# tkortz/opencv

Hardware: AMD Instinct MI355X
Metric: tracked frames/sec, 1080p×128-object TBD loop @ 1/2/4/8 MI355X (higher is better)
Workload: dtype u8; 1 GPU; TBD loop 1920x1080 x 128 objects (BASELINE configs[2]), frames [5, 2577) of a 2577-frame sequence per GPU; levels=3, win=21, gftt=256/box, q 0.01, minDist 3, every 5, tracker_bounds=reference, parallelism=replicas x1 (one sequence per GPU), api=tbdk_tbd_run (native frame loop, look-ahead)

## Files before the change

opencv_amd/csrc/klt_gftt.hip:

```cpp
#include <atomic>
#include <cfloat>
#include <cmath>
#include <type_traits>

#include "klt_gftt_device.hpp"
#include "tbdk_internal.hpp"

namespace tbdk {

namespace {

__device__ __forceinline__ int refl(int p, int len)
{
    if ((unsigned)p < (unsigned)len) return p;
    if (len == 1) return 0;
    do {
        if (p < 0) p = -p;
        else p = 2 * len - 2 - p;
    } while ((unsigned)p >= (unsigned)len);
    return p;
}

}

__device__ __forceinline__ int roi_of_cblock(const GfttArgs& a, int b)
{
    int lo = 0, hi = a.nroi - 1;
    while (lo < hi) {
        const int mid = (lo + hi + 1) >> 1;
        if ((a.ninl > 0 ? a.inl[mid].cblk : a.rois[mid].cblk) <= b) lo = mid;
        else hi = mid - 1;
    }
    return lo;
}

__device__ __forceinline__ float from_left(float v)
{
    return __int_as_float(__builtin_amdgcn_mov_dpp(__float_as_int(v), 0x138, 0xF, 0xF, true));
}
__device__ __forceinline__ float from_right(float v)
{
    return __int_as_float(__builtin_amdgcn_mov_dpp(__float_as_int(v), 0x130, 0xF, 0xF, true));
}

struct SobelRow {
    float rx, ry;
};
__device__ __forceinline__ SobelRow sobel_row(float s0, float s1, float s2, float k, float k2)
{
    float t = -1.f * s0;
    t = t + 0.f * s1;
    t = t + 1.f * s2;
    float u = k * s0;
    u = u + k2 * s1;
    u = u + k * s2;
    return SobelRow{t, u};
}
__device__ __forceinline__ SobelRow sobel_row_f32(float s0, float s1, float s2, float k, float k2)
{
    return SobelRow{s2 - s0, s1 * k2 + (s0 + s2) * k};
}

#ifndef TBDK_GFTT_EIG_WAVES
#define TBDK_GFTT_EIG_WAVES 4
#endif
constexpr int kEigWaves = TBDK_GFTT_EIG_WAVES;
constexpr int kEigPref = 8;
#ifndef TBDK_GFTT_EIG_PREF_C
#define TBDK_GFTT_EIG_PREF_C 4
#endif
#ifndef TBDK_GFTT_WALK_PRIO
#define TBDK_GFTT_WALK_PRIO 3
#endif
#ifndef GFTT_ESTAMP
#define GFTT_ESTAMP(i)
#endif

struct EigLane {
    __amdgpu_buffer_rsrc_t rs;
    int x, H, hm2, pitch;
    bool mir, out_lane;
    float k, k2;
};

__device__ __forceinline__ uint32_t row_off(int row, int pitch) { return (uint32_t)row * (uint32_t)pitch; }

struct EigMask {
    __amdgpu_buffer_rsrc_t rs;
    uint32_t col;
    int pitch;
};
__device__ __forceinline__ bool eig_mask_ld(const EigMask& m, int row)
{
    return __builtin_amdgcn_raw_buffer_load_b8(m.rs, m.col, (int)row_off(row, m.pitch), 0) != 0;
}

template <int PX = TBDK_PIX_U8>
__device__ __forceinline__ float eig_ld(const EigLane& g, int row)
{
    if constexpr (PX == TBDK_PIX_F32)
        return __uint_as_float(__builtin_amdgcn_raw_buffer_load_b32(g.rs, g.x * 4, (int)row_off(row, g.pitch), 0));
    else if constexpr (PX == TBDK_PIX_U16)
        return (float)__builtin_amdgcn_raw_buffer_load_b16(g.rs, g.x * 2, (int)row_off(row, g.pitch), 0);
    else
        return (float)__builtin_amdgcn_raw_buffer_load_b8(g.rs, g.x, (int)row_off(row, g.pitch), 0);
}

template <int PX = TBDK_PIX_U8>
__device__ __forceinline__ SobelRow eig_srow(const EigLane& g, float v)
{
    const float l = from_left(v), rr = from_right(v);
    if constexpr (PX != TBDK_PIX_U8) return sobel_row_f32(g.mir ? rr : l, v, g.mir ? l : rr, g.k, g.k2);
    else return sobel_row(g.mir ? rr : l, v, g.mir ? l : rr, g.k, g.k2);
}

__device__ __forceinline__ void eig_rowsums(const EigLane& g, const SobelRow& p, const SobelRow& c,
                                            const SobelRow& n, double (&out)[3])
{
    const float dx = (p.rx + n.rx) * g.k + (c.rx * g.k2 + 0.f);
    const float dy = (n.ry - p.ry) + 0.f;
    const float cv[3] = {dx * dx, dx * dy, dy * dy};
#pragma unroll
    for (int ch = 0; ch < 3; ++ch) {
        const float l = from_left(cv[ch]), rr = from_right(cv[ch]);
        out[ch] = (double)l + (double)cv[ch] + (double)rr;
    }
}

template <bool compact, bool masked, int PREF = compact ? TBDK_GFTT_EIG_PREF_C : kEigPref, int PX = TBDK_PIX_U8>
__device__ __forceinline__ void eig_segment(const EigLane& g, const EigMask& gm, float* __restrict__ E,
                                            uint64_t* __restrict__ lm,
                                            int w, int ep, int y0, int y1, int ys, int ye, int ycap, bool fresh,
                                            double (&S)[3], double (&S0)[3], double (&Scap)[3], int& best, int ccol)
{
    const int H = g.H;
    auto pix = [&](int yy) { return eig_ld<PX>(g, refl(yy, H)); };
    auto pix_fwd = [&](int yy) { return eig_ld<PX>(g, yy < H ? yy : g.hm2); };
    const int lane = threadIdx.x & 63;
    const bool x_in = g.out_lane && g.x >= 1 && g.x <= w - 2;
    double qa[3], qb[3];
    {
        const int rm = refl(ys - 1, H);
        eig_rowsums(g, eig_srow<PX>(g, pix(rm - 1)), eig_srow<PX>(g, pix(rm)), eig_srow<PX>(g, pix(rm + 1)), qa);
    }
    SobelRow wa = eig_srow<PX>(g, pix(ys)), wb = eig_srow<PX>(g, pix(ys + 1));
    eig_rowsums(g, eig_srow<PX>(g, pix(ys - 1)), wa, wb, qb);
    if (fresh) {
#pragma unroll
        for (int ch = 0; ch < 3; ++ch) S[ch] = (0.0 + qa[ch]) + qb[ch];
    }
#pragma unroll
    for (int ch = 0; ch < 3; ++ch) S0[ch] = S[ch];
    float e1 = 0.f, e2 = 0.f;
    const __amdgpu_buffer_rsrc_t rE =
        __builtin_amdgcn_make_buffer_rsrc(E - g.x, (short)0, ep * H * 4, 0x00020000);
    const __amdgpu_buffer_rsrc_t rL = __builtin_amdgcn_make_buffer_rsrc(lm, (short)0, lm ? H * 8 : 0, 0x00020000);
    constexpr uint32_t kDrop = 0x80000000u;
    const uint32_t eoff = g.out_lane ? (uint32_t)g.x * 4u : kDrop;
    auto row = [&](auto steady, int y, float cur, bool has_next, bool store, bool lmx) {
        constexpr bool ST = decltype(steady)::value;
        bool m_in = true;
        if constexpr (masked) {
            if (ST || store) m_in = eig_mask_ld(gm, y);
        }
        double in[3];
        SobelRow wc = wb;
        if (ST || has_next) {
            wc = eig_srow<PX>(g, cur);
            eig_rowsums(g, wa, wb, wc, in);
        } else {
#pragma unroll
            for (int ch = 0; ch < 3; ++ch) in[ch] = qa[ch];
        }
        float box[3];
#pragma unroll
        for (int ch = 0; ch < 3; ++ch) {
            const double t = S[ch] + in[ch];
            box[ch] = (float)t;
            S[ch] = t - qa[ch];
            qa[ch] = qb[ch];
            qb[ch] = in[ch];
        }
        wa = wb;
        wb = wc;
        const float aa = box[0] * 0.5f, bb = box[1], cc = box[2] * 0.5f;
        const float t = aa - cc;
        const float e = (aa + cc) - sqrtf(bb * bb + t * t);
        if (ST || store) {
            if constexpr (!compact)
                __builtin_amdgcn_raw_buffer_store_b32(__float_as_uint(e), rE, eoff == kDrop ? kDrop : eoff + (uint32_t)(y * ep * 4), 0, 0);
            const int kk = fkey(e);
            if constexpr (masked) best = (g.out_lane && m_in && kk > best) ? kk : best;
            else best = (g.out_lane && kk > best) ? kk : best;
        }
        if (ST || lmx) {
            float m = fmaxf(e2, e);
            m = fmaxf(m, fmaxf(from_left(e2), from_right(e2)));
            m = fmaxf(m, fmaxf(from_left(e1), from_right(e1)));
            m = fmaxf(m, fmaxf(from_left(e), from_right(e)));
            const bool lmax = x_in && e1 >= m;
            const uint64_t bal = __ballot(lmax);
            typedef unsigned int u32x2 __attribute__((ext_vector_type(2)));
            const u32x2 bv = {(unsigned)bal, (unsigned)(bal >> 32)};
            __builtin_amdgcn_raw_buffer_store_b64(bv, rL, lane == 0 ? (uint32_t)((y - 1) * 8) : kDrop, 0, 0);
            if constexpr (compact) {
                const uint32_t rk =
                    __builtin_amdgcn_mbcnt_hi((unsigned)(bal >> 32), __builtin_amdgcn_mbcnt_lo((unsigned)bal, 0u));
                __builtin_amdgcn_raw_buffer_store_b32(__float_as_uint(e1), rE,
                                                      lmax ? (uint32_t)(((y - 1) * ep + ccol + (int)rk) * 4) : kDrop, 0, 0);
            }
        }
        e2 = e1;
        e1 = e;
    };
    auto generic = [&](int y) {
        if (y == ycap) {
#pragma unroll
            for (int ch = 0; ch < 3; ++ch) Scap[ch] = S[ch];
        }
        const int yc = y - 1;
        row(std::false_type{}, y, y + 1 < H ? pix_fwd(y + 2) : 0.f, y + 1 < H, y >= y0 && y < y1,
            yc >= y0 && yc < y1 && yc >= 1 && yc <= H - 2);
    };
    const int sa = max(max(y0 + 1, 2), ys);
    int sb = min(min(y1, H - 1), ye);
    if (ycap >= 0) sb = min(sb, ycap);
    int y = ys;
    if (sb - sa >= PREF) {
        for (; y < sa; ++y) generic(y);
        float nxt[PREF];
#pragma unroll
        for (int j = 0; j < PREF; ++j) nxt[j] = pix_fwd(y + 2 + j);
        for (; y + PREF <= sb; y += PREF) {
            float cur[PREF];
#pragma unroll
            for (int j = 0; j < PREF; ++j) cur[j] = nxt[j];
#pragma unroll
            for (int j = 0; j < PREF; ++j) nxt[j] = pix_fwd(min(y + PREF + 2 + j, H));
#pragma unroll
            for (int j = 0; j < PREF; ++j) row(std::true_type{}, y + j, cur[j], true, true, true);
        }
    }
    for (; y < ye; ++y) generic(y);
}

template <bool compact, bool masked, int PX = TBDK_PIX_U8>
__device__ __forceinline__ void gftt_eig_body(const GfttArgs& a)
{
    constexpr int kPref = compact ? TBDK_GFTT_EIG_PREF_C : kEigPref;
    constexpr int kBpp = PX == TBDK_PIX_F32 ? 4 : PX == TBDK_PIX_U16 ? 2 : 1;
    __shared__ double s_cap[kEigWaves][3][64];
    __shared__ double s_drift[3][64];
    __shared__ int s_best[kEigWaves];
    __shared__ int s_bad;
    const int r = roi_of_cblock(a, blockIdx.x);
    const GfttRoi R = roi_at(a, r);
    const int wv = __builtin_amdgcn_readfirstlane(threadIdx.x >> 6);
    const int lane = threadIdx.x & 63;
    const int H = R.h;

    EigLane g;
    const int strip = blockIdx.x - R.cblk;
    const int xc = strip * kGfttStrip - kGfttHalo + lane;
    g.out_lane = lane >= kGfttHalo && lane < kGfttHalo + kGfttStrip && xc < R.w;
    {
        const int w = R.w;
        int xm = xc < -2 || xc > w + 1 ? min(max(xc, 0), w - 1) : xc;
        if (w == 1) {
            xm = 0;
        } else {
#pragma unroll
            for (int it = 0; it < 2; ++it) {
                if (xm < 0) xm = -xm;
                if (xm >= w) xm = 2 * (w - 1) - xm;
            }
        }
        g.x = xm;
        g.mir = xc < 0 || xc >= w;
    }
    const double scale = PX == TBDK_PIX_U8 ? 1.0 / ((double)(1 << 2) * 3 * 255.0) : 1.0 / ((double)(1 << 2) * 3);
    g.k = (float)(1.0 * scale);
    g.k2 = (float)(2.0 * scale);
    g.H = H;
    g.hm2 = H >= 2 ? H - 2 : 0;
    g.pitch = a.pitch;
    g.rs = __builtin_amdgcn_make_buffer_rsrc(const_cast<uint8_t*>(a.img + (size_t)R.y * a.pitch + (size_t)R.x * kBpp),
                                             (short)0, (int)(row_off(H - 1, a.pitch) + (uint32_t)(R.w * kBpp)),
                                             0x00020000);
    EigMask gm{};
    if constexpr (masked) {
        gm.rs = __builtin_amdgcn_make_buffer_rsrc(const_cast<uint8_t*>(a.mask + (size_t)R.y * a.mask_pitch + R.x),
                                                  (short)0, (int)(row_off(H - 1, a.mask_pitch) + (uint32_t)R.w),
                                                  0x00020000);
        gm.col = g.out_lane ? (uint32_t)g.x : 0xFFFFFFFFu;
        gm.pitch = a.mask_pitch;
    }
    float* E = a.eig + R.off + g.x;
    uint64_t* lm = a.lmax + R.moff + (size_t)strip * H;
    const bool has_lm = R.w >= 3 && H >= 3;
    const int ccol = strip * kGfttStrip;

    const int L = (H + kEigWaves - 1) / kEigWaves;
    const int y0 = wv * L, y1 = min(H, y0 + L);
    const bool live = y0 < y1;
    const int ys = y0 > 0 ? y0 - 1 : 0, ye = min(H, y1 + 1);
    const int ycap = y1 < H ? y1 - 1 : -1;
    int best = INT_MIN;
    double S[3], S0[3], Scap[3];
    const bool need = lane >= kGfttHalo - 1 && lane <= kGfttHalo + kGfttStrip && xc >= 0 && xc < R.w;
    auto first_mismatch = [&](int from) {
        if (threadIdx.x == 0) s_bad = kEigWaves;
        __syncthreads();
        if (live && wv > from) {
            bool diff = a.eig_redo != 0 && wv == from + 1;
#pragma unroll
            for (int ch = 0; ch < 3; ++ch) diff |= need && S0[ch] != s_cap[wv - 1][ch][lane];
            if (__any(diff) && lane == 0) atomicMin(&s_bad, wv);
        }
        __syncthreads();
        return s_bad;
    };
    GFTT_ESTAMP(0);
    if (live) {
        eig_segment<compact, masked, kPref, PX>(g, gm, E, has_lm ? lm : nullptr, R.w, gftt_epitch(R.w), y0, y1, ys, ye,
                                                ycap, true, S, S0, Scap, best, ccol);
        if (ycap >= 0) {
#pragma unroll
            for (int ch = 0; ch < 3; ++ch) s_cap[wv][ch][lane] = Scap[ch];
        }
    }
    int bad = first_mismatch(0);
    GFTT_ESTAMP(1);
    while (bad < kEigWaves) {
        if (wv == bad && live) {
#pragma unroll
            for (int ch = 0; ch < 3; ++ch) s_drift[ch][lane] = s_cap[bad - 1][ch][lane] - S0[ch];
        }
        __syncthreads();
        if (wv >= bad && live) {
#pragma unroll
            for (int ch = 0; ch < 3; ++ch)
                S[ch] = wv == bad ? s_cap[bad - 1][ch][lane] : S0[ch] + s_drift[ch][lane];
        }
        __syncthreads();
        if (wv >= bad && live) {
            best = INT_MIN;
            eig_segment<compact, masked, kPref, PX>(g, gm, E, has_lm ? lm : nullptr, R.w, gftt_epitch(R.w), y0, y1, ys,
                                                    ye, ycap, false, S, S0, Scap, best, ccol);
            if (ycap >= 0) {
#pragma unroll
                for (int ch = 0; ch < 3; ++ch) s_cap[wv][ch][lane] = Scap[ch];
            }
        }
        bad = first_mismatch(bad);
    }
#pragma unroll
    for (int o = 32; o > 0; o >>= 1) {
        const int v = __shfl_xor(best, o);
        best = v > best ? v : best;
    }
    if (lane == 0) s_best[wv] = best;
    __syncthreads();
    GFTT_ESTAMP(2);
    if (threadIdx.x == 0) {
        int m = s_best[0];
#pragma unroll
        for (int k = 1; k < kEigWaves; ++k) m = s_best[k] > m ? s_best[k] : m;
        a.blk_max[blockIdx.x] = m;
    }
}

template <bool compact>
__global__ __launch_bounds__(64 * kEigWaves) void gftt_eig_kernel(GfttArgs a)
{
    gftt_eig_body<compact, false>(a);
}

template <bool compact>
__global__ __launch_bounds__(64 * kEigWaves) void gftt_eig_masked_kernel(GfttArgs a)
{
    gftt_eig_body<compact, true>(a);
}

template <bool compact, bool masked, int PX>
__global__ __launch_bounds__(64 * kEigWaves) void gftt_eigpx_kernel(GfttArgs a)
{
    static_assert(PX == TBDK_PIX_U16 || PX == TBDK_PIX_F32, "the 8-bit kernels are gftt_eig_kernel / gftt_eig_masked_kernel");
    gftt_eig_body<compact, masked, PX>(a);
}

#ifndef GFTT_STAMP
#define GFTT_STAMP(i)
#define GFTT_TDECL
#define GFTT_T(i)
#define GFTT_TDUMP
#endif

template <int J>
__device__ __forceinline__ int xor_lane(int v, int lane)
{
    if constexpr (J == 1) return __builtin_amdgcn_mov_dpp(v, 0xB1, 0xF, 0xF, true);
    else if constexpr (J == 2) return __builtin_amdgcn_mov_dpp(v, 0x4E, 0xF, 0xF, true);
    else if constexpr (J == 4 || J == 8) {
        const int up = __builtin_amdgcn_mov_dpp(v, 0x100 | J, 0xF, 0xF, true);
        const int dn = __builtin_amdgcn_mov_dpp(v, 0x110 | J, 0xF, 0xF, true);
        return (lane & J) ? dn : up;
    } else if constexpr (J == 16) return __builtin_amdgcn_ds_swizzle(v, 0x1F | (16 << 10));
    else return __shfl_xor(v, J);
}
template <int J>
__device__ __forceinline__ uint64_t xor_lane_u64(uint64_t v, int lane)
{
    const int lo = xor_lane<J>((int)(uint32_t)v, lane), hi = xor_lane<J>((int)(uint32_t)(v >> 32), lane);
    return ((uint64_t)(uint32_t)hi << 32) | (uint32_t)lo;
}

__device__ __forceinline__ void sort_keys_512(uint64_t* keys, int tid)
{
    static_assert(kSelThreads == 512, "eight runs of 64");
    const int lane = tid & 63, w = tid >> 6;
    uint64_t x = keys[tid];
    auto stage = [&](auto jc, int k) {
        constexpr int j = decltype(jc)::value;
        const uint64_t y = xor_lane_u64<j>(x, lane);
        const bool desc = (lane & k) == 0 || k == 64;
        const bool take_max = ((lane & j) == 0) == desc;
        x = take_max ? (x > y ? x : y) : (x < y ? x : y);
    };
    using I1 = std::integral_constant<int, 1>;
    using I2 = std::integral_constant<int, 2>;
    using I4 = std::integral_constant<int, 4>;
    using I8 = std::integral_constant<int, 8>;
    using I16 = std::integral_constant<int, 16>;
    using I32 = std::integral_constant<int, 32>;
    stage(I1{}, 2);
    stage(I2{}, 4), stage(I1{}, 4);
    stage(I4{}, 8), stage(I2{}, 8), stage(I1{}, 8);
    stage(I8{}, 16), stage(I4{}, 16), stage(I2{}, 16), stage(I1{}, 16);
    stage(I16{}, 32), stage(I8{}, 32), stage(I4{}, 32), stage(I2{}, 32), stage(I1{}, 32);
    stage(I32{}, 64), stage(I16{}, 64), stage(I8{}, 64), stage(I4{}, 64), stage(I2{}, 64), stage(I1{}, 64);
    keys[tid] = x;
    __syncthreads();
    int rank = lane;
    int pos[8];
    bool all[8];
#pragma unroll
    for (int r = 0; r < 8; ++r) {
        const uint64_t c = keys[r * 64 + 63];
        all[r] = r < w ? c >= x : c > x;
        pos[r] = 0;
    }
#pragma unroll
    for (int st = 32; st >= 1; st >>= 1) {
#pragma unroll
        for (int r = 0; r < 8; ++r) {
            const uint64_t c = keys[r * 64 + pos[r] + st - 1];
            const bool ahead = r < w ? c >= x : c > x;
            pos[r] += ahead ? st : 0;
        }
    }
#pragma unroll
    for (int r = 0; r < 8; ++r) rank += r != w ? (all[r] ? 64 : pos[r]) : 0;
    __syncthreads();
    keys[rank] = x;
    __syncthreads();
}

template <int RAD>
__device__ __forceinline__ void window_test(const uint8_t* img, int rw, int rh, int ix, int iy, float fx, float fy,
                                            int lane, double md2, bool& good, unsigned long long& inb)
{
    constexpr int NR = 2 * RAD + 1;
    constexpr bool THREE = NR + 7 > 16;
    constexpr uint64_t kHi = 0x8080808080808080ull, kLo7 = 0x7F7F7F7F7F7F7F7Full;
    const int x0 = ix - RAD;
    if constexpr (RAD <= 2) {
        uint64_t cv = 0;
#pragma unroll
        for (int t = 0; t < NR; ++t) {
            const int xx = x0 + t;
            cv |= ((xx >= 0 && xx < rw) ? 0xFFull : 0ull) << (8 * t);
        }
        uint64_t wv[NR];
        int sh[NR];
#pragma unroll
        for (int d = 0; d < NR; ++d) {
            const int yy = iy - RAD + d;
            const int yc = yy < 0 ? 0 : (yy >= rh ? rh - 1 : yy);
            const int base = yc * rw + x0;
            const int al = base > 0 ? (base & ~3) : 0;
            const uint32_t* wp = reinterpret_cast<const uint32_t*>(img + al);
            wv[d] = (uint64_t)wp[0] | ((uint64_t)wp[1] << 32);
            sh[d] = base - al;
        }
        uint64_t rej = 0;
#pragma unroll
        for (int d = 0; d < NR; ++d) {
            const int yy = iy - RAD + d;
            if (yy < 0 || yy >= rh) continue;
            uint64_t close = 0;
#pragma unroll
            for (int t = 0; t < NR; ++t) {
                const float ddx = (float)(t - RAD), ddy = (float)(d - RAD);
                close |= (((double)(ddx * ddx + ddy * ddy) < md2 && !(d == RAD && t == RAD)) ? 0xFFull : 0ull)
                         << (8 * t);
            }
            const uint64_t v = (sh[d] >= 0 ? wv[d] >> (8 * sh[d]) : wv[d] << (-8 * sh[d])) & cv & close;
            rej |= v & kHi;
            uint64_t nz = (((v & kLo7) + kLo7) | v) & ~v & kHi;
            while (nz) {
                const int t = __builtin_ctzll(nz) >> 3;
                nz &= nz - 1ull;
                const int c = (int)((v >> (8 * t)) & 0xFF);
                if (c - 1 < lane) inb |= 1ull << (c - 1);
            }
        }
        if (rej) good = false;
        (void)fx;
        (void)fy;
        return;
    }
    uint64_t cv_lo = 0, cv_hi = 0;
#pragma unroll
    for (int t = 0; t < NR; ++t) {
        const int xx = x0 + t;
        const uint64_t b = (xx >= 0 && xx < rw) ? 0xFFull : 0ull;
        if (t < 8) cv_lo |= b << (8 * t);
        else cv_hi |= b << (8 * (t - 8));
    }
    uint64_t w0[NR], w1[NR], w2[NR];
    int sh[NR];
#pragma unroll
    for (int d = 0; d < NR; ++d) {
        const int yy = iy - RAD + d;
        const int yc = yy < 0 ? 0 : (yy >= rh ? rh - 1 : yy);
        const int base = yc * rw + x0;
        const int al = base > 0 ? (base & ~7) : 0;
        const uint64_t* wp = reinterpret_cast<const uint64_t*>(img + al);
        w0[d] = wp[0];
        w1[d] = wp[1];
        w2[d] = THREE ? wp[2] : 0ull;
        sh[d] = base - al;
    }
    uint64_t rej = 0;
#pragma unroll
    for (int d = 0; d < NR; ++d) {
        const int yy = iy - RAD + d;
        if (yy < 0 || yy >= rh) continue;
        uint64_t close_lo = 0, close_hi = 0;
#pragma unroll
        for (int t = 0; t < NR; ++t) {
            const float ddx = (float)(t - RAD), ddy = (float)(d - RAD);
            const uint64_t b = ((double)(ddx * ddx + ddy * ddy) < md2 && !(d == RAD && t == RAD)) ? 0xFFull : 0ull;
            if (t < 8) close_lo |= b << (8 * t);
            else close_hi |= b << (8 * (t - 8));
        }
        uint64_t lo, hi;
        if (sh[d] >= 0) {
            const int b8 = 8 * sh[d];
            lo = sh[d] ? (w0[d] >> b8) | (w1[d] << (64 - b8)) : w0[d];
            hi = sh[d] ? (w1[d] >> b8) | (w2[d] << (64 - b8)) : w1[d];
        } else {
            const int b8 = -8 * sh[d];
            lo = w0[d] << b8;
            hi = (w1[d] << b8) | (w0[d] >> (64 - b8));
        }
        lo &= cv_lo & close_lo;
        hi &= cv_hi & close_hi;
        rej |= (lo | hi) & kHi;
        uint64_t nz_lo = (((lo & kLo7) + kLo7) | lo) & ~lo & kHi;
        uint64_t nz_hi = (((hi & kLo7) + kLo7) | hi) & ~hi & kHi;
        while (nz_lo | nz_hi) {
            int t;
            uint64_t src;
            if (nz_lo) {
                t = __builtin_ctzll(nz_lo) >> 3;
                nz_lo &= nz_lo - 1ull;
                src = lo;
            } else {
                t = __builtin_ctzll(nz_hi) >> 3;
                nz_hi &= nz_hi - 1ull;
                src = hi;
                t += 8;
            }
            const int v = (int)((src >> (8 * (t & 7))) & 0xFF);
            if (v - 1 < lane) inb |= 1ull << (v - 1);
        }
    }
    if (rej) good = false;
    (void)fx;
    (void)fy;
}

#ifndef TBDK_GFTT_PARTIAL
#define TBDK_GFTT_PARTIAL 1
#endif
constexpr int kSelTarget = 448;
constexpr int kSelRegs = 8;

__device__ uint64_t take_next64(uint64_t* rest, int nrest, int lane)
{
    uint64_t mine = 0ull;
    for (int c = 0; c < 64; ++c) {
        uint64_t best = 0ull;
        int bi = -1;
        for (int j = lane; j < nrest; j += 64) {
            const uint64_t v = rest[j];
            if (v > best) {
                best = v;
                bi = j;
            }
        }
        uint64_t m = best;
#pragma unroll
        for (int d = 32; d >= 1; d >>= 1) {
            const uint64_t o = shfl_xor_u64(m, d);
            m = o > m ? o : m;
        }
        if (m == 0ull) break;
        if (bi >= 0 && best == m) rest[bi] = 0ull;
        if (lane == c) mine = m;
        __builtin_amdgcn_s_waitcnt(0xC07F);
        __builtin_amdgcn_wave_barrier();
    }
    return mine;
}

template <int RMAX, bool masked = false>
__global__ __launch_bounds__(kSelThreads) void gftt_select_kernel(GfttArgs a)
{
    extern __shared__ __attribute__((aligned(16))) uint8_t smem[];
    uint64_t* keys = reinterpret_cast<uint64_t*>(smem);
    float2* acc = reinterpret_cast<float2*>(keys + a.cap);
    float2* bxy = acc + a.max_corners;
    uint8_t* img = reinterpret_cast<uint8_t*>(acc + ((a.max_corners + 65) & ~1));
    const int r = blockIdx.x;
    const GfttRoi R = roi_at(a, r);
    const int tid = threadIdx.x;
    __shared__ int s_total;
    GFTT_STAMP(0);
    const int area = R.w * R.h;
    const bool use_dist = a.min_distance >= 1.0;
    const double md2 = a.min_distance * a.min_distance;
    int rad = (int)ceil(a.min_distance) - 1;
    if ((double)(rad + 1) * (rad + 1) < md2) rad++;
    const bool img_mode = use_dist && area <= a.img_bytes && rad <= 6;
    if (img_mode)
        for (int i = tid * 16; i < area; i += kSelThreads * 16) *reinterpret_cast<uint4*>(img + i) = make_uint4(0, 0, 0, 0);

    const int nstrip = (R.w + kGfttStrip - 1) / kGfttStrip;
    const int nw = R.w >= 3 && R.h >= 3 ? nstrip * R.h : 0;
    const uint64_t word0 = tid < nw ? a.lmax[R.moff + tid] : 0ull;
    int mk = INT_MIN;
    {
        int b = R.cblk;
        const int e = R.cblk + nstrip;
        for (; b + 4 <= e; b += 4) {
            const int m0 = a.blk_max[b], m1 = a.blk_max[b + 1], m2 = a.blk_max[b + 2], m3 = a.blk_max[b + 3];
            mk = max(max(mk, max(m0, m1)), max(m2, m3));
        }
        for (; b < e; ++b) mk = a.blk_max[b] > mk ? a.blk_max[b] : mk;
    }
    const float roi_max = masked && mk == INT_MIN ? 0.f : fkey_inv(mk);
    const float thr = (float)((double)roi_max * a.quality);
    if (tid == 0) s_total = 0;
    __syncthreads();
    const float* Ep = a.eig + R.off;
    const uint8_t* Mp = masked ? a.mask + (size_t)R.y * a.mask_pitch + R.x : nullptr;
    if (R.w >= 3 && R.h >= 3) {
        if (thr > 0.f) {
            for (int wi = tid; wi < nw; wi += kSelThreads) {
                const int st = wi / R.h, y = wi - st * R.h;
                if (y < 1 || y > R.h - 2) continue;
                uint64_t word = wi == tid ? word0 : a.lmax[R.moff + wi];
                const float* Er = Ep + (size_t)y * gftt_epitch(R.w) + st * kGfttStrip - kGfttHalo;
                const float* Ec = Er + kGfttHalo;
                const uint8_t* Mr = masked ? Mp + (size_t)y * a.mask_pitch + st * kGfttStrip - kGfttHalo : nullptr;
                int rk = 0;
                while (word) {
                    int xs[8];
                    float vs[8];
                    [[maybe_unused]] uint8_t ms[8];
#pragma unroll
                    for (int u = 0; u < 8; ++u) {
                        xs[u] = -1;
                        if (word) {
                            xs[u] = __builtin_ctzll(word);
                            word &= word - 1ull;
                            vs[u] = a.compact ? Ec[rk++] : Er[xs[u]];
                            if constexpr (masked) ms[u] = Mr[xs[u]];
                        }
                    }
#pragma unroll
                    for (int u = 0; u < 8; ++u) {
                        bool in = xs[u] >= 0 && vs[u] > thr;
                        if constexpr (masked) in = in && ms[u] != 0;
                        if (in) {
                            const int q = atomicAdd(&s_total, 1);
                            if (q < a.cap) keys[q] = cand_key(vs[u], y, st * kGfttStrip + xs[u] - kGfttHalo);
                        }
                    }
                }
            }
        } else if (!a.compact) {
            const int iw = R.w - 2, n = iw * (R.h - 2), ep = gftt_epitch(R.w);
            for (int p = tid; p < n; p += kSelThreads) {
                const int y = p / iw + 1, x = p - (y - 1) * iw + 1;
                const float* Ec = Ep + (size_t)y * ep + x;
                const float v = Ec[0] > thr ? Ec[0] : 0.f;
                if (v == 0.f) continue;
                if constexpr (masked) {
                    if (Mp[(size_t)y * a.mask_pitch + x] == 0) continue;
                }
                float m = v;
#pragma unroll
                for (int dy = -1; dy <= 1; ++dy)
#pragma unroll
                    for (int dx = -1; dx <= 1; ++dx) {
                        const float q0 = Ec[dy * ep + dx];
                        const float q = q0 > thr ? q0 : 0.f;
                        m = q > m ? q : m;
                    }
                if (v == m) {
                    const int q = atomicAdd(&s_total, 1);
                    if (q < a.cap) keys[q] = cand_key(v, y, x);
                }
            }
        }
    }
    __syncthreads();
    GFTT_STAMP(4);
    const int total = s_total;
    if (total > a.cap) {
        if (tid == 0) a.counts[r] = -1;
        return;
    }
    int S = total, nrest = 0;
    if (TBDK_GFTT_PARTIAL && total > kSelThreads && total <= kSelRegs * kSelThreads && total + kSelThreads + 64 <= a.cap) {
        __shared__ int hist[256];
        __shared__ int s_pick[4];
        __shared__ int s_cnt[2];
        if (tid < 256) hist[tid] = 0;
        __syncthreads();
        for (int i = tid; i < total; i += kSelThreads) atomicAdd(&hist[(int)(keys[i] >> 56)], 1);
        __syncthreads();
        if (tid < 64) radix_pick(hist, kSelTarget, tid, &s_pick[0], &s_pick[1]);
        __syncthreads();
        const int b1 = s_pick[0], above1 = s_pick[1];
        if (tid < 256) hist[tid] = 0;
        __syncthreads();
        for (int i = tid; i < total; i += kSelThreads) {
            const uint64_t k = keys[i];
            if ((int)(k >> 56) == b1) atomicAdd(&hist[(int)(k >> 48) & 255], 1);
        }
        __syncthreads();
        if (tid < 64) {
            int b2 = -1, above2 = 0;
            radix_pick(hist, kSelTarget - above1, tid, &b2, &above2);
            if (b2 >= 0) {
                s_pick[2] = (b1 << 8) | b2;
                s_pick[3] = above1 + above2 + hist[b2];
            }
        }
        if (tid == 0) s_cnt[0] = s_cnt[1] = 0;
        __syncthreads();
        const int sel = s_pick[3];
        if (sel <= kSelThreads) {
            const uint32_t t16 = (uint32_t)s_pick[2];
            uint64_t kr[kSelRegs];
#pragma unroll
            for (int u = 0; u < kSelRegs; ++u) {
                const int i = tid + u * kSelThreads;
                kr[u] = i < total ? keys[i] : 0ull;
            }
            __syncthreads();
#pragma unroll
            for (int u = 0; u < kSelRegs; ++u) {
                if (tid + u * kSelThreads >= total) continue;
                if ((uint32_t)(kr[u] >> 48) >= t16) keys[atomicAdd(&s_cnt[0], 1)] = kr[u];
                else keys[kSelThreads + atomicAdd(&s_cnt[1], 1)] = kr[u];
            }
            __syncthreads();
            S = sel;
            nrest = total - sel;
        }
    }
    GFTT_STAMP(5);
    int np2 = kSelThreads;
    while (np2 < S) np2 <<= 1;
    for (int i = S + tid; i < np2; i += kSelThreads) keys[i] = 0ull;
    __syncthreads();
    GFTT_STAMP(1);
    switch (np2 / kSelThreads) {
    case 1: sort_keys_512(keys, tid); break;
    case 2: sort_keys<2>(keys, np2, tid); break;
    case 4: sort_keys<4>(keys, np2, tid); break;
    default: sort_keys_lds(keys, np2, tid); break;
    }
    GFTT_STAMP(2);
    if (tid >= 64) return;
    __builtin_amdgcn_s_setprio(TBDK_GFTT_WALK_PRIO);

    const int lane = tid;
    const int maxc = a.max_corners;
    float2* out = a.corners + (size_t)r * a.corner_stride;
    int n = 0;
    bool done = false;
    GFTT_TDECL;
    int i0 = 0, rem = nrest;
    while (!done) {
        GFTT_T(0);
        uint64_t key;
        bool valid;
        if (i0 < S) {
            const int i = i0 + lane;
            valid = i < S;
            key = valid ? keys[i] : 0ull;
            i0 += 64;
        } else {
            if (rem <= 0) break;
            key = take_next64(keys + kSelThreads, nrest, lane);
            valid = key != 0ull;
            rem -= 64;
        }
        const uint32_t kk = (uint32_t)key;
        const int ix = (int)(kk & 0xFFFF), iy = (int)(kk >> 16);
        const float fx = (float)ix, fy = (float)iy;
        bool good = valid;
        unsigned long long inb = 0ull;
        if (img_mode) {
            if (valid) img[iy * R.w + ix] = (uint8_t)(lane + 1);
            __builtin_amdgcn_s_waitcnt(0xC07F);
            __builtin_amdgcn_wave_barrier();
            GFTT_T(1);
            if (valid) {
                switch (rad) {
                case 0: window_test<0>(img, R.w, R.h, ix, iy, fx, fy, lane, md2, good, inb); break;
                case 1: window_test<1>(img, R.w, R.h, ix, iy, fx, fy, lane, md2, good, inb); break;
                case 2: window_test<2>(img, R.w, R.h, ix, iy, fx, fy, lane, md2, good, inb); break;
                default:
                    if constexpr (RMAX > 2) {
                        switch (rad) {
                        case 3: window_test<3>(img, R.w, R.h, ix, iy, fx, fy, lane, md2, good, inb); break;
                        case 4: window_test<4>(img, R.w, R.h, ix, iy, fx, fy, lane, md2, good, inb); break;
                        case 5: window_test<5>(img, R.w, R.h, ix, iy, fx, fy, lane, md2, good, inb); break;
                        default: window_test<6>(img, R.w, R.h, ix, iy, fx, fy, lane, md2, good, inb); break;
                        }
                    }
                    break;
                }
            }
        } else if (use_dist) {
            bxy[lane] = make_float2(fx, fy);
            for (int q = 0; q < n && good; ++q) {
                const float2 pq = acc[q];
                const float dx = fx - pq.x, dy = fy - pq.y;
                if ((double)(dx * dx + dy * dy) < md2) good = false;
            }
            __builtin_amdgcn_s_waitcnt(0xC07F);
            __builtin_amdgcn_wave_barrier();
            for (int j = 0; j < lane; ++j) {
                const float2 pj = bxy[j];
                const float dx = fx - pj.x, dy = fy - pj.y;
                if ((double)(dx * dx + dy * dy) < md2) inb |= 1ull << j;
            }
        }
        GFTT_T(2);
        const unsigned long long goodm = __ballot(good);
        const unsigned long long depm = __ballot(good && inb != 0ull);
        unsigned long long accm = goodm & ~depm;
        unsigned long long pend = depm;
        while (pend) {
            const int k = __builtin_ctzll(pend);
            pend &= pend - 1ull;
            const unsigned long long ik =
                ((unsigned long long)(uint32_t)__builtin_amdgcn_readlane((int)(inb >> 32), k) << 32) |
                (uint32_t)__builtin_amdgcn_readlane((int)(uint32_t)inb, k);
            if (!(ik & accm)) accm |= 1ull << k;
        }
        GFTT_T(3);
        const int got = __popcll(accm);
        if (n + got >= maxc) {
            int keepn = maxc - n;
            unsigned long long m = accm, t = 0ull;
            while (keepn-- > 0) {
                const unsigned long long low = m & (~m + 1ull);
                t |= low;
                m &= m - 1ull;
            }
            accm = t;
            done = true;
        }
        GFTT_T(4);
        const bool mine = (accm >> lane) & 1ull;
        if (mine) {
            const int pos = n + __popcll(accm & ((1ull << lane) - 1ull));
            if (!img_mode) acc[pos] = make_float2(fx, fy);
            out[pos] = make_float2(fx + (float)R.x, fy + (float)R.y);
        }
        if (img_mode && valid) img[iy * R.w + ix] = mine ? (uint8_t)255 : (uint8_t)0;
        n += __popcll(accm);
        __builtin_amdgcn_s_waitcnt(0xC07F);
        __builtin_amdgcn_wave_barrier();
        GFTT_T(5);
    }
    GFTT_TDUMP;
    GFTT_STAMP(3);
    if (lane == 0) a.counts[r] = n;
}

size_t gftt_select_smem(int cap, int max_corners, int img_bytes)
{
    return sizeof(uint64_t) * (size_t)cap +
           sizeof(float2) * (size_t)((max_corners + 65) & ~1) + (size_t)img_bytes + 32;
}

void gftt_plan(GfttArgs& a, int max_area)
{
    const long lds = 160L * 1024 - 2048;
    const long fixed = (long)gftt_select_smem(0, a.max_corners, 0);
    long img = ((long)max_area + 15) & ~15L;
    long room = lds - fixed - img;
    if (room < 8L * 4096) {
        img = 0;
        room = lds - fixed;
    }
    int cap = 512;
    while (cap < kGfttCap && 8L * cap * 2 <= room) cap <<= 1;
    a.cap = cap;
    a.img_bytes = (int)img;
}

template <int PX>
static void launch_gftt_eigpx(const GfttArgs& a, dim3 grid, dim3 block, hipStream_t s)
{
    if (a.mask) {
        if (a.compact) hipLaunchKernelGGL((gftt_eigpx_kernel<true, true, PX>), grid, block, 0, s, a);
        else hipLaunchKernelGGL((gftt_eigpx_kernel<false, true, PX>), grid, block, 0, s, a);
    } else {
        if (a.compact) hipLaunchKernelGGL((gftt_eigpx_kernel<true, false, PX>), grid, block, 0, s, a);
        else hipLaunchKernelGGL((gftt_eigpx_kernel<false, false, PX>), grid, block, 0, s, a);
    }
}

hipError_t launch_gftt_eig(const GfttArgs& a, hipStream_t s, int pix)
{
    const dim3 grid(a.ncblk), block(64 * kEigWaves);
    if (pix == TBDK_PIX_F32) {
        launch_gftt_eigpx<TBDK_PIX_F32>(a, grid, block, s);
    } else if (pix == TBDK_PIX_U16) {
        launch_gftt_eigpx<TBDK_PIX_U16>(a, grid, block, s);
    } else if (a.mask) {
        if (a.compact) hipLaunchKernelGGL(gftt_eig_masked_kernel<true>, grid, block, 0, s, a);
        else hipLaunchKernelGGL(gftt_eig_masked_kernel<false>, grid, block, 0, s, a);
    } else {
        if (a.compact) hipLaunchKernelGGL(gftt_eig_kernel<true>, grid, block, 0, s, a);
        else hipLaunchKernelGGL(gftt_eig_kernel<false>, grid, block, 0, s, a);
    }
    return hipGetLastError();
}

hipError_t launch_gftt(const GfttArgs& a, hipStream_t s, hipEvent_t after_eig, int pix, bool select)
{
    const hipError_t e0 = launch_gftt_eig(a, s, pix);
    if (e0 != hipSuccess) return e0;
    if (after_eig) {
        const hipError_t e = hipEventRecord(after_eig, s);
        if (e != hipSuccess) return e;
    }
    return select ? launch_gftt_select(a, s) : hipSuccess;
}

hipError_t launch_gftt_select(const GfttArgs& a, hipStream_t s)
{
    const size_t smem = gftt_select_smem(a.cap, a.max_corners, a.img_bytes);
    static std::atomic<unsigned long long> opted{0};
    int dev = 0;
    hipError_t e = hipGetDevice(&dev);
    if (e != hipSuccess) return e;
    const unsigned long long bit = 1ull << (dev & 63);
    if (!(opted.load(std::memory_order_acquire) & bit)) {
        for (const void* k : {reinterpret_cast<const void*>(&gftt_select_kernel<2>),
                              reinterpret_cast<const void*>(&gftt_select_kernel<6>),
                              reinterpret_cast<const void*>(&gftt_select_kernel<2, true>),
                              reinterpret_cast<const void*>(&gftt_select_kernel<6, true>)}) {
            hipFuncAttributes fa;
            e = hipFuncGetAttributes(&fa, k);
            if (e != hipSuccess) return e;
            e = hipFuncSetAttribute(k, hipFuncAttributeMaxDynamicSharedMemorySize,
                                    (int)(160L * 1024 - (long)fa.sharedSizeBytes));
            if (e != hipSuccess) return e;
        }
        opted.fetch_or(bit, std::memory_order_acq_rel);
    }
    const double md2 = a.min_distance * a.min_distance;
    int rad = (int)ceil(a.min_distance) - 1;
    if ((double)(rad + 1) * (rad + 1) < md2) rad++;
    const bool wide = a.min_distance >= 1.0 && rad > 2;
    if (a.mask) {
        if (wide) hipLaunchKernelGGL((gftt_select_kernel<6, true>), dim3(a.nroi), dim3(kSelThreads), smem, s, a);
        else hipLaunchKernelGGL((gftt_select_kernel<2, true>), dim3(a.nroi), dim3(kSelThreads), smem, s, a);
    } else if (wide)
        hipLaunchKernelGGL(gftt_select_kernel<6>, dim3(a.nroi), dim3(kSelThreads), smem, s, a);
    else
        hipLaunchKernelGGL(gftt_select_kernel<2>, dim3(a.nroi), dim3(kSelThreads), smem, s, a);
    return hipGetLastError();
}

}
```

Baseline: 6420 frames/s.

## Streamline GFTT eigen kernel: reuse row max, float best, scalar offsets, tail loop

Moves the Sobel/gradient/eigenvalue helpers into a shared host/device header and simplifies the integer-pixel arithmetic by dropping the zero-literal terms. The 3x3 local-max test now reuses a per-row horizontal max (hmax3) carried across rows instead of recomputing six DPP moves per row. The unmasked best score is tracked as a float and keyed once at the end. Buffer offsets move into the scalar soffset slot and ROI fields are forced uniform with readfirstlane. A remainder loop lets the prefetched steady-state path handle segments shorter than the prefetch depth. The risk is small numeric differences from reassociated integer-path math and more complex control flow.

Measured after the change: 6729 frames/s (median of 6 runs). +4.8%, better.

```diff
diff --git a/opencv_amd/csrc/gftt_row_math.hpp b/opencv_amd/csrc/gftt_row_math.hpp
--- /dev/null
+++ b/opencv_amd/csrc/gftt_row_math.hpp
@@ -0,0 +1,62 @@
+#pragma once
+#include <cmath>
+
+#if defined(__HIPCC__)
+#include <hip/hip_runtime.h>
+#define TBDK_ROW_HD __host__ __device__ __forceinline__
+#else
+#define TBDK_ROW_HD inline
+#endif
+
+namespace tbdk {
+
+struct SobelRow {
+    float rx, ry;
+};
+
+TBDK_ROW_HD SobelRow sobel_row_lit(float s0, float s1, float s2, float k, float k2)
+{
+    float t = -1.f * s0;
+    t = t + 0.f * s1;
+    t = t + 1.f * s2;
+    float u = k * s0;
+    u = u + k2 * s1;
+    u = u + k * s2;
+    return SobelRow{t, u};
+}
+
+TBDK_ROW_HD SobelRow sobel_row(float s0, float s1, float s2, float k, float k2)
+{
+    float u = k * s0;
+    u = u + k2 * s1;
+    u = u + k * s2;
+    return SobelRow{s2 - s0, u};
+}
+
+TBDK_ROW_HD SobelRow sobel_row_f32(float s0, float s1, float s2, float k, float k2)
+{
+    return SobelRow{s2 - s0, s1 * k2 + (s0 + s2) * k};
+}
+
+struct Grad {
+    float dx, dy;
+};
+TBDK_ROW_HD Grad grad_lit(const SobelRow& p, const SobelRow& c, const SobelRow& n, float k, float k2)
+{
+    return Grad{(p.rx + n.rx) * k + (c.rx * k2 + 0.f), (n.ry - p.ry) + 0.f};
+}
+TBDK_ROW_HD Grad grad_int(const SobelRow& p, const SobelRow& c, const SobelRow& n, float k, float k2)
+{
+    return Grad{(p.rx + n.rx) * k + c.rx * k2, n.ry - p.ry};
+}
+
+TBDK_ROW_HD float min_eig(float a, float b, float c)
+{
+    const float aa = a * 0.5f, bb = b, cc = c * 0.5f;
+    const float t = aa - cc;
+    return (aa + cc) - sqrtf(bb * bb + t * t);
+}
+
+TBDK_ROW_HD int fkey_bits(int i) { return i >= 0 ? i : i ^ 0x7FFFFFFF; }
+
+}
diff --git a/opencv_amd/csrc/klt_gftt.hip b/opencv_amd/csrc/klt_gftt.hip
--- a/opencv_amd/csrc/klt_gftt.hip
+++ b/opencv_amd/csrc/klt_gftt.hip
@@ -3,6 +3,7 @@
 #include <cmath>
 #include <type_traits>
 
+#include "gftt_row_math.hpp"
 #include "klt_gftt_device.hpp"
 #include "tbdk_internal.hpp"
 
@@ -43,23 +44,8 @@
     return __int_as_float(__builtin_amdgcn_mov_dpp(__float_as_int(v), 0x130, 0xF, 0xF, true));
 }
 
-struct SobelRow {
-    float rx, ry;
-};
-__device__ __forceinline__ SobelRow sobel_row(float s0, float s1, float s2, float k, float k2)
-{
-    float t = -1.f * s0;
-    t = t + 0.f * s1;
-    t = t + 1.f * s2;
-    float u = k * s0;
-    u = u + k2 * s1;
-    u = u + k * s2;
-    return SobelRow{t, u};
-}
-__device__ __forceinline__ SobelRow sobel_row_f32(float s0, float s1, float s2, float k, float k2)
-{
-    return SobelRow{s2 - s0, s1 * k2 + (s0 + s2) * k};
-}
+__device__ __forceinline__ float hmax3(float v) { return fmaxf(fmaxf(v, from_left(v)), from_right(v)); }
+
 
 #ifndef TBDK_GFTT_EIG_WAVES
 #define TBDK_GFTT_EIG_WAVES 4
@@ -114,11 +100,12 @@
     else return sobel_row(g.mir ? rr : l, v, g.mir ? l : rr, g.k, g.k2);
 }
 
+template <int PX = TBDK_PIX_U8>
 __device__ __forceinline__ void eig_rowsums(const EigLane& g, const SobelRow& p, const SobelRow& c,
                                             const SobelRow& n, double (&out)[3])
 {
-    const float dx = (p.rx + n.rx) * g.k + (c.rx * g.k2 + 0.f);
-    const float dy = (n.ry - p.ry) + 0.f;
+    const Grad gr = PX == TBDK_PIX_F32 ? grad_lit(p, c, n, g.k, g.k2) : grad_int(p, c, n, g.k, g.k2);
+    const float dx = gr.dx, dy = gr.dy;
     const float cv[3] = {dx * dx, dx * dy, dy * dy};
 #pragma unroll
     for (int ch = 0; ch < 3; ++ch) {
@@ -141,25 +128,30 @@
     double qa[3], qb[3];
     {
         const int rm = refl(ys - 1, H);
-        eig_rowsums(g, eig_srow<PX>(g, pix(rm - 1)), eig_srow<PX>(g, pix(rm)), eig_srow<PX>(g, pix(rm + 1)), qa);
+        eig_rowsums<PX>(g, eig_srow<PX>(g, pix(rm - 1)), eig_srow<PX>(g, pix(rm)), eig_srow<PX>(g, pix(rm + 1)), qa);
     }
     SobelRow wa = eig_srow<PX>(g, pix(ys)), wb = eig_srow<PX>(g, pix(ys + 1));
-    eig_rowsums(g, eig_srow<PX>(g, pix(ys - 1)), wa, wb, qb);
+    eig_rowsums<PX>(g, eig_srow<PX>(g, pix(ys - 1)), wa, wb, qb);
     if (fresh) {
 #pragma unroll
         for (int ch = 0; ch < 3; ++ch) S[ch] = (0.0 + qa[ch]) + qb[ch];
     }
 #pragma unroll
     for (int ch = 0; ch < 3; ++ch) S0[ch] = S[ch];
+    constexpr bool HLM = PX != TBDK_PIX_F32;
+    constexpr bool FBEST = !masked && PX != TBDK_PIX_F32;
     float e1 = 0.f, e2 = 0.f;
+    float h1 = 0.f, h2 = 0.f;
+    float bestf = -INFINITY;
     const __amdgpu_buffer_rsrc_t rE =
-        __builtin_amdgcn_make_buffer_rsrc(E - g.x, (short)0, ep * H * 4, 0x00020000);
+        __builtin_amdgcn_make_buffer_rsrc(E, (short)0, ep * H * 4, 0x00020000);
     const __amdgpu_buffer_rsrc_t rL = __builtin_amdgcn_make_buffer_rsrc(lm, (short)0, lm ? H * 8 : 0, 0x00020000);
     constexpr uint32_t kDrop = 0x80000000u;
     const uint32_t eoff = g.out_lane ? (uint32_t)g.x * 4u : kDrop;
+    const uint32_t loff = lane == 0 ? 0u : kDrop;
     auto row = [&](auto steady, int y, float cur, bool has_next, bool store, bool lmx) {
         constexpr bool ST = decltype(steady)::value;
-        bool m_in = true;
+        [[maybe_unused]] bool m_in = true;
         if constexpr (masked) {
             if (ST || store) m_in = eig_mask_ld(gm, y);
         }
@@ -167,7 +159,7 @@
         SobelRow wc = wb;
         if (ST || has_next) {
             wc = eig_srow<PX>(g, cur);
-            eig_rowsums(g, wa, wb, wc, in);
+            eig_rowsums<PX>(g, wa, wb, wc, in);
         } else {
 #pragma unroll
             for (int ch = 0; ch < 3; ++ch) in[ch] = qa[ch];
@@ -183,35 +175,45 @@
         }
         wa = wb;
         wb = wc;
-        const float aa = box[0] * 0.5f, bb = box[1], cc = box[2] * 0.5f;
-        const float t = aa - cc;
-        const float e = (aa + cc) - sqrtf(bb * bb + t * t);
+        const float e = min_eig(box[0], box[1], box[2]);
         if (ST || store) {
-            if constexpr (!compact)
-                __builtin_amdgcn_raw_buffer_store_b32(__float_as_uint(e), rE, eoff == kDrop ? kDrop : eoff + (uint32_t)(y * ep * 4), 0, 0);
-            const int kk = fkey(e);
-            if constexpr (masked) best = (g.out_lane && m_in && kk > best) ? kk : best;
-            else best = (g.out_lane && kk > best) ? kk : best;
-        }
+            if constexpr (!compact) __builtin_amdgcn_raw_buffer_store_b32(__float_as_uint(e), rE, eoff, y * ep * 4, 0);
+            if constexpr (FBEST) {
+                bestf = fmaxf(bestf, e);
+            } else {
+                const int kk = fkey(e);
+                if constexpr (masked) best = (g.out_lane && m_in && kk > best) ? kk : best;
+                else best = (g.out_lane && kk > best) ? kk : best;
+            }
+        }
+        float h = 0.f;
+        if constexpr (HLM) h = hmax3(e);
         if (ST || lmx) {
-            float m = fmaxf(e2, e);
-            m = fmaxf(m, fmaxf(from_left(e2), from_right(e2)));
-            m = fmaxf(m, fmaxf(from_left(e1), from_right(e1)));
-            m = fmaxf(m, fmaxf(from_left(e), from_right(e)));
+            float m;
+            if constexpr (HLM) {
+                m = fmaxf(fmaxf(h2, h1), h);
+            } else {
+                m = fmaxf(e2, e);
+                m = fmaxf(m, fmaxf(from_left(e2), from_right(e2)));
+                m = fmaxf(m, fmaxf(from_left(e1), from_right(e1)));
+                m = fmaxf(m, fmaxf(from_left(e), from_right(e)));
+            }
             const bool lmax = x_in && e1 >= m;
             const uint64_t bal = __ballot(lmax);
             typedef unsigned int u32x2 __attribute__((ext_vector_type(2)));
             const u32x2 bv = {(unsigned)bal, (unsigned)(bal >> 32)};
-            __builtin_amdgcn_raw_buffer_store_b64(bv, rL, lane == 0 ? (uint32_t)((y - 1) * 8) : kDrop, 0, 0);
+            __builtin_amdgcn_raw_buffer_store_b64(bv, rL, loff, (y - 1) * 8, 0);
             if constexpr (compact) {
                 const uint32_t rk =
                     __builtin_amdgcn_mbcnt_hi((unsigned)(bal >> 32), __builtin_amdgcn_mbcnt_lo((unsigned)bal, 0u));
-                __builtin_amdgcn_raw_buffer_store_b32(__float_as_uint(e1), rE,
-                                                      lmax ? (uint32_t)(((y - 1) * ep + ccol + (int)rk) * 4) : kDrop, 0, 0);
+                __builtin_amdgcn_raw_buffer_store_b32(__float_as_uint(e1), rE, lmax ? rk * 4u : kDrop,
+                                                      ((y - 1) * ep + ccol) * 4, 0);
             }
         }
         e2 = e1;
         e1 = e;
+        h2 = h1;
+        h1 = h;
     };
     auto generic = [&](int y) {
         if (y == ycap) {
@@ -226,11 +228,11 @@
     int sb = min(min(y1, H - 1), ye);
     if (ycap >= 0) sb = min(sb, ycap);
     int y = ys;
-    if (sb - sa >= PREF) {
+    if (sb > sa) {
         for (; y < sa; ++y) generic(y);
         float nxt[PREF];
 #pragma unroll
-        for (int j = 0; j < PREF; ++j) nxt[j] = pix_fwd(y + 2 + j);
+        for (int j = 0; j < PREF; ++j) nxt[j] = pix_fwd(min(y + 2 + j, H));
         for (; y + PREF <= sb; y += PREF) {
             float cur[PREF];
 #pragma unroll
@@ -240,8 +242,18 @@
 #pragma unroll
             for (int j = 0; j < PREF; ++j) row(std::true_type{}, y + j, cur[j], true, true, true);
         }
+        float cur = nxt[0];
+        for (; y < sb; ++y) {
+            const float nx = pix_fwd(min(y + 3, H));
+            row(std::true_type{}, y, cur, true, true, true);
+            cur = nx;
+        }
     }
     for (; y < ye; ++y) generic(y);
+    if constexpr (FBEST) {
+        const int kk = fkey(bestf);
+        best = (g.out_lane && kk > best) ? kk : best;
+    }
 }
 
 template <bool compact, bool masked, int PX = TBDK_PIX_U8>
@@ -254,7 +266,9 @@
     __shared__ int s_best[kEigWaves];
     __shared__ int s_bad;
     const int r = roi_of_cblock(a, blockIdx.x);
-    const GfttRoi R = roi_at(a, r);
+    const GfttRoi Rv = roi_at(a, r);
+    auto uni = [](int v) { return __builtin_amdgcn_readfirstlane(v); };
+    const GfttRoi R{uni(Rv.x), uni(Rv.y), uni(Rv.w), uni(Rv.h), uni(Rv.off), uni(Rv.moff), uni(Rv.cblk)};
     const int wv = __builtin_amdgcn_readfirstlane(threadIdx.x >> 6);
     const int lane = threadIdx.x & 63;
     const int H = R.h;
@@ -295,7 +309,7 @@
         gm.col = g.out_lane ? (uint32_t)g.x : 0xFFFFFFFFu;
         gm.pitch = a.mask_pitch;
     }
-    float* E = a.eig + R.off + g.x;
+    float* E = a.eig + R.off;
     uint64_t* lm = a.lmax + R.moff + (size_t)strip * H;
     const bool has_lm = R.w >= 3 && H >= 3;
     const int ccol = strip * kGfttStrip;
@@ -345,8 +359,12 @@
         __syncthreads();
         if (wv >= bad && live) {
             best = INT_MIN;
-            eig_segment<compact, masked, kPref, PX>(g, gm, E, has_lm ? lm : nullptr, R.w, gftt_epitch(R.w), y0, y1, ys,
-                                                    ye, ycap, false, S, S0, Scap, best, ccol);
+            int c0 = y0;
+            asm volatile("" : "+s"(c0));
+            const int c1 = min(H, c0 + L);
+            eig_segment<compact, masked, kPref, PX>(g, gm, E, has_lm ? lm : nullptr, R.w, gftt_epitch(R.w), c0, c1,
+                                                    c0 > 0 ? c0 - 1 : 0, min(H, c1 + 1), c1 < H ? c1 - 1 : -1, false, S,
+                                                    S0, Scap, best, ccol);
             if (ycap >= 0) {
 #pragma unroll
                 for (int ch = 0; ch < 3; ++ch) s_cap[wv][ch][lane] = Scap[ch];
```
